# Nikhil-AI-Labs/image-super-resolution-2

Measured on AMD Instinct MI355X. Metric: output MPix/s at x4 SR (256->1024), higher is better.
Workload: dtype bf16 (bf16 MFMA operands, fp32 accumulate, fp32 activations in HBM); 1 GPU; FreqFusion x4 full 3-expert forward (HAT-L + DAT + NAFNet-SR + fusion stack), one 256x256 LR tile -> 1024x1024 per step per GPU (BASELINE configs[1]); seeded synthetic weights (172.3 M params), 1/f-noise tiles; tile=256, parallelism=tile-sharded x1, weights RCCL-broadcast once (0.0 ms), no per-tile collectives, launch=hipGraph replay, tiles_in_flight=2

## Files before the change

image-super-resolution-2_amd/build.py:

```python
from __future__ import annotations

import os
import subprocess
import sys
from concurrent.futures import ThreadPoolExecutor

HERE = os.path.dirname(os.path.abspath(__file__))
CSRC = os.path.join(HERE, "csrc")
LIB = os.path.join(HERE, "libff_hip.so")
SOURCES = ["ff_runtime.hip", "conv_gemm.hip", "conv_gemm_bf16.hip", "conv3x3_halo.hip", "sgfn_tail.hip", "ocab_attn.hip", "conv3x3_small.hip", "attention.hip", "attention_bf16.hip", "win_attn_fused.hip", "chan_qkv.hip", "token_mlp.hip", "token_linear.hip", "naf_fused.hip", "norm_pool.hip", "dwconv.hip", "elementwise.hip",
           "resample.hip", "freq.hip", "fusion_ops.hip", "metrics.hip", "train_ops.hip", "sr_losses.hip", "ff_executor.hip"]
HIPCC = os.environ.get("HIPCC", "/opt/rocm/bin/hipcc")
FLAGS = ["--offload-arch=gfx950", "-O3", "-fPIC", "-std=c++17", "-Wall", "-Wno-unused-function", "-I" + os.path.join(HERE, "build")]


def _stale() -> bool:
    if not os.path.exists(LIB):
        return True
    t = os.path.getmtime(LIB)
    deps = [os.path.join(CSRC, f) for f in os.listdir(CSRC)] + [os.path.join(HERE, "..", "include", "ff_kernels.h")]
    return any(os.path.getmtime(d) > t for d in deps)


def gen_dispatch(path: str) -> None:
    from .lib import parse_header
    protos = {n: p for n, p in parse_header().items() if p[1] and p[1][-1] == "void*" and p[0] == "int"
              and n not in ("ff_forward", "ff_create", "ff_upload")}
    names = sorted(protos)
    out = ["// generated by build.py from include/ff_kernels.h -- do not edit", f"#define FF_DISPATCH_COUNT {len(names)}",
           "static const char* const FF_DISPATCH_NAMES[FF_DISPATCH_COUNT] = {" + ", ".join(f'"{n}"' for n in names) + "};"]
    def kinds(n):
        ks = []
        for i, ty in enumerate(protos[n][1]):
            if i == len(protos[n][1]) - 1:
                ks.append("S")
            elif ty.endswith("*"):
                ks.append("P")
            elif ty in ("float", "double"):
                ks.append("F")
            else:
                ks.append("I")
        return "".join(ks)
    out.append("static const char* const FF_DISPATCH_KINDS[FF_DISPATCH_COUNT] = {" + ", ".join(f'"{kinds(n)}"' for n in names) + "};")
    for n in names:
        out.append(f'extern "C" int {n}(' + ", ".join(protos[n][1]) + ");")
    out.append("static int ff_dispatch(int id, const FFVal* v) {\n  switch (id) {")
    for k, n in enumerate(names):
        args = []
        for i, ty in enumerate(protos[n][1]):
            if ty.endswith("*"):
                args.append(f"({ty})v[{i}].p")
            elif ty in ("float", "double"):
                args.append(f"({ty})v[{i}].f")
            else:
                args.append(f"({ty})v[{i}].i")
        out.append(f"    case {k}: return {n}(" + ", ".join(args) + ");")
    out.append('    default: ff_set_error("ff_dispatch: bad entry point id %d", id); return FF_ERR_ARG;\n  }\n}')
    txt = "\n".join(out) + "\n"
    if not os.path.exists(path) or open(path).read() != txt:
        open(path, "w").write(txt)


def build(force: bool = False, verbose: bool = False) -> str:
# ... 27 lines not shown
```

image-super-resolution-2_amd/experts.py:

```python
from __future__ import annotations

import os
from typing import Dict, List, Optional

import torch

from . import ops
from .prep import (pack_conv, pack_dw, bn_scale_shift, fold_bn_after_conv, pack_token_mlp, pack_token_linear, pack_naf_ffn,
                   pack_win_attn, pack_win_rel, pack_token_projmlp, pack_chan_qkv, pack_token_linear_gated, pack_rel_overlap)

T = torch.Tensor
SD = Dict[str, T]
RGB_MEAN = (0.4488, 0.4371, 0.4040)


def _ceil_to(n: int, m: int) -> int:
    return (n + m - 1) // m * m


class _Weights:

    def __init__(self, sd: SD, dev, prefix: str):
        self.sd, self.dev, self.p = sd, dev, prefix

    def __call__(self, name: str) -> T:
        return self.sd[self.p + name].to(self.dev, torch.float32).contiguous()

    def conv(self, name: str) -> T:
        return pack_conv(self(name + ".weight"))

    def opt(self, name: str) -> Optional[T]:
        k = self.p + name
        return self.sd[k].to(self.dev, torch.float32).contiguous() if k in self.sd else None


def _tl(blk: dict, key: str) -> dict:
    pk = blk.get(key + "_tl")
    if pk is None:
        pk = blk[key + "_tl"] = pack_token_linear(blk[key][0], blk[key][1])
    return pk


_BF16_ROWS = os.environ.get("FF_BF16_ROWS", "1") != "0"
_OCAB_V2 = os.environ.get("FF_OCAB_V2", "1") != "0"
_SGFN_TAIL = os.environ.get("FF_SGFN_TAIL", "1") != "0"


def _fast() -> bool:
    return ops.fused_modes()


_WIN_FUSED = os.environ.get("FF_WIN_FUSED", "1") != "0"
_PROJ_MLP = os.environ.get("FF_PROJ_MLP", "1") != "0"
_LN_ON_LOAD = os.environ.get("FF_LN_ON_LOAD", "1") != "0"
_CHAN_FUSED = os.environ.get("FF_CHAN_FUSED", "1") != "0"
_GATED_PROJ = os.environ.get("FF_GATED_PROJ", "1") != "0"


def _pm(blk: dict) -> dict:
    pk = blk.get("projmlp_pk")
    if pk is None:
# ... 365 lines not shown
            x = ops.conv2d(x, *self.after, ksize=(3, 3), pad=(1, 1), res=feat)
        x = ops.conv2d(x, *self.before_up, ksize=(3, 3), pad=(1, 1), act="lrelu")
        x = ops.conv2d(x, *self.up0, ksize=(3, 3), pad=(1, 1), shuffle=2)
        x = ops.conv2d(x, *self.up2, ksize=(3, 3), pad=(1, 1), shuffle=2)
        sr = ops.conv2d(x, *self.last, ksize=(3, 3), pad=(1, 1))
        return ops.nhwc_to_nchw(sr, 4 * h, 4 * w, clamp01=True)


class NafnetHIP:

    def __init__(self, sd: SD, dev, prefix: str = "expert_ensemble.nafnet.nafnet.", enc=(2, 2, 4, 8), mid: int = 12,
                 dec=(2, 2, 2, 2)):
        w = _Weights(sd, dev, prefix)
        self.dev, self.enc_n, self.mid_n, self.dec_n = dev, enc, mid, dec

        def blk(q):
            def c1(n):
                wt = w(q + n + ".weight")
                return wt.reshape(wt.shape[0], wt.shape[1]).contiguous(), w(q + n + ".bias")
            return dict(n1=(w(q + "norm1.weight"), w(q + "norm1.bias")), n2=(w(q + "norm2.weight"), w(q + "norm2.bias")),
                        c1=c1("conv1"), c2=(pack_dw(w(q + "conv2.weight")), w(q + "conv2.bias")), c3=c1("conv3"),
                        sca=c1("sca.1"), c4=c1("conv4"), c5=c1("conv5"),
                        beta=w(q + "beta").reshape(-1).contiguous(), gamma=w(q + "gamma").reshape(-1).contiguous())

        self.intro = (w.conv("intro"), w("intro.bias"))
        self.ending = (w.conv("ending"), w("ending.bias"))
        self.encs = [[blk(f"encoders.{l}.{b}.") for b in range(n)] for l, n in enumerate(enc)]
        self.mids = [blk(f"middle_blks.{b}.") for b in range(mid)]
        self.decs = [[blk(f"decoders.{l}.{b}.") for b in range(n)] for l, n in enumerate(dec)]
        self.downs = [(w.conv(f"downs.{l}"), w(f"downs.{l}.bias")) for l in range(len(enc))]
        self.ups = [w(f"ups.{l}.0.weight").reshape(w(f"ups.{l}.0.weight").shape[0], -1).contiguous() for l in range(len(dec))]

    def _padded_input(self, B: int, Hp: int, Wp: int, dev) -> T:
        return ops.persistent_zeros(id(self), "naf_in", (B, Hp, Wp, 3), dev)

    def __del__(self):
        try:
            ops.drop_persistent(owner=id(self))
        except Exception:
            pass

    def block(self, x: T, k: dict) -> T:
        c = x.shape[-1]
        flash = _fast() and c in (64, 128)
        if flash and _NAF_FRONT and c == 64:
            g, pooled = ops.naf_front(x, _tl(k, "c1"), k["n1"][0], k["n1"][1], *k["c2"])
        else:
            if flash:
                t = ops.token_linear(x, _tl(k, "c1"), gamma=k["n1"][0], beta=k["n1"][1], eps=1e-6)
            else:
                t = ops.linear(ops.layernorm(x, *k["n1"], eps=1e-6), *k["c1"])
            g, pooled = ops.dwconv3_gate_pool(t, *k["c2"])
        sca = ops.vec_mlp(pooled, *k["sca"], None)
        nf = ops.gemm_mode() != "f32"
        if nf:
            y = ops.linear(g, *k["c3"], res=x, mul=k["beta"], kmul=sca.reshape(-1))
        else:
            w3 = ops.mix2(k["c3"][0], ca=sca.reshape(-1))
            y = ops.linear(g, w3, k["c3"][1], res=x, mul=k["beta"], dynamic_w=True)
        if flash:
            if "ffn_pk" not in k:
                k["ffn_pk"] = pack_naf_ffn(k["c4"][0], k["c4"][1], k["c5"][0], k["c5"][1])
            return ops.naf_ffn(y, k["ffn_pk"], k["n2"][0], k["n2"][1], k["gamma"])
        if nf:
            if "c4i" not in k:
                w4, b4 = k["c4"]
                k["c4i"] = (torch.stack((w4[:c], w4[c:]), dim=1).reshape(2 * c, -1).contiguous(),
                            torch.stack((b4[:c], b4[c:]), dim=1).reshape(-1).contiguous())
            g = ops.linear(ops.layernorm(y, *k["n2"], eps=1e-6), *k["c4i"], gate_pairs=True)
        else:
            t = ops.linear(ops.layernorm(y, *k["n2"], eps=1e-6), *k["c4"])
            g = ops.fma3(None, t[..., :c], t[..., c:])
        return ops.linear(g, *k["c5"], res=y, mul=k["gamma"])

    def forward(self, lr: T, taps: Optional[dict] = None, feats: Optional[dict] = None) -> T:
        _, _, h, w = lr.shape
        H, W = 4 * h, 4 * w
        m = 2 ** len(self.enc_n)
        Hp, Wp = _ceil_to(H, m), _ceil_to(W, m)
        inp = self._padded_input(1, Hp, Wp, lr.device)
        ops.resize(lr, (H, W), mode="bicubic", scale_factor=4.0, layout="nchw", out=inp)
        x = ops.conv2d(inp, *self.intro, ksize=(3, 3), pad=(1, 1))
        skips = []
        for lvl, blks in enumerate(self.encs):
            for b, k in enumerate(blks):
                x = self.block(x, k)
                if taps is not None and lvl == 0:
                    taps[f"naf.enc0.b{b}"] = x
            skips.append(x)
            x = ops.conv2d(x, *self.downs[lvl], ksize=(2, 2), stride=(2, 2), pad=(0, 0))
        for k in self.mids:
            x = self.block(x, k)
        if taps is not None:
            taps["naf.mid"] = x
        for lvl, blks in enumerate(self.decs):
            x = ops.conv2d(x, self.ups[lvl], None, shuffle=2, res=skips[-1 - lvl])
            for k in blks:
                x = self.block(x, k)
        if feats is not None:
            feats["nafnet"] = x
        x = ops.conv2d(x, *self.ending, ksize=(3, 3), pad=(1, 1), res=inp)
        return ops.nhwc_to_nchw(x, H, W, clamp01=True)
```

image-super-resolution-2_amd/ops.py:

```python
from __future__ import annotations

from typing import Dict, Optional, Tuple

import torch

from . import lib as _lib

ACT = {None: 0, "none": 0, "gelu": 1, "relu": 2, "lrelu": 3, "sigmoid": 4}
T = torch.Tensor

_PROF = None
_META = [0.0, 0.0]


def _note(flops: float = 0.0, nbytes: float = 0.0):
    _META[0] += flops
    _META[1] += nbytes


def _numel(*ts) -> float:
    return float(sum(t.numel() * (t.element_size() / 4.0) for t in ts if t is not None))


def _instrument(fn):
# ... 544 lines not shown
        slo, shi = stats_range
        stats = torch.empty((rows, 2), device=x.device, dtype=torch.float32)
        sp = stats.data_ptr()
    _lib.check(_L().ff_token_linear(xp, ldx, out.data_ptr(), ldo, rows, K, pk["kpad"], N, pk["nt"], _ptr(gamma), _ptr(beta), float(eps),
                                    pk["w"].data_ptr(), _ptr(pk["b"]), ACT[act], rp, ldr, r2p, ldr2, _ptr(res2_scale), xnp, ldxn,
                                    sp, slo, shi, float(stats_eps), _nterms(), _stream()))
    _note(2.0 * rows * N * K, 4.0 * (rows * K * (2 if want_xn else 1) + rows * N * (1 + (res is not None) + (res2 is not None))))
    if stats is not None:
        return out, stats
    return (out, xn) if want_xn else out


def dwconv3_gate_pool(t: T, w_tap: T, bias: T):
    tp, ldi, B, H, W, C2 = _nhwc(t, "dwconv3_gate_pool.t")
    if B != 1 or C2 % 2 or tuple(w_tap.shape) != (9, C2):
        raise _lib.FFError("dwconv3_gate_pool: expects B == 1, [9, 2C] tap-major weights")
    C = C2 // 2
    out = torch.empty((1, H, W, C), device=t.device, dtype=torch.float32)
    pooled = torch.empty((1, C), device=t.device, dtype=torch.float32)
    nwork = int(_L().ff_dwconv3_gate_pool_workspace(C))
    work = torch.empty(nwork, device=t.device, dtype=torch.float32)
    _lib.check(_L().ff_dwconv3_gate_pool(tp, ldi, out.data_ptr(), C, H, W, C, w_tap.data_ptr(), bias.data_ptr(), pooled.data_ptr(),
                                         work.data_ptr(), nwork, _stream()))
    _note(2.0 * H * W * C2 * 9, 4.0 * H * W * (C2 + C))
    return out, pooled


def naf_front(x: T, pk: dict, ln_g: T, ln_b: T, w_tap: T, dw_bias: T, eps: float = 1e-6):
    xp, ldx, B, H, W, C = _nhwc(x, "naf_front.x")
    if B != 1 or C not in (64, 128) or pk["N"] != 2 * C or pk["K"] != C or pk["kpad"] != C or tuple(w_tap.shape) != (9, 2 * C):
        raise _lib.FFError("naf_front: expects B == 1, C in (64, 128), conv1 packed as [2C, C], [9, 2C] tap-major weights")
    out = torch.empty((1, H, W, C), device=x.device, dtype=torch.float32)
    pooled = torch.empty((1, C), device=x.device, dtype=torch.float32)
    nwork = int(_L().ff_naf_front_workspace(H, W, C))
    work = torch.empty(nwork, device=x.device, dtype=torch.float32)
    _lib.check(_L().ff_naf_front(xp, ldx, H, W, C, ln_g.data_ptr(), ln_b.data_ptr(), float(eps), pk["w"].data_ptr(), pk["b"].data_ptr(),
                                 w_tap.data_ptr(), dw_bias.data_ptr(), out.data_ptr(), C, pooled.data_ptr(), work.data_ptr(), nwork,
                                 _nterms(), _stream()))
    _note(2.0 * H * W * 2 * C * (C + 9), 4.0 * H * W * 2 * C)
    return out, pooled


def naf_ffn(y: T, pk: dict, ln_g: T, ln_b: T, out_scale: T, eps: float = 1e-6) -> T:
    yp, ldy, rows, C = rows_view(y, "naf_ffn.y")
    if C != pk["C"]:
        raise _lib.FFError("naf_ffn: channel mismatch")
    out = torch.empty(tuple(y.shape), device=y.device, dtype=torch.float32)
    _lib.check(_L().ff_naf_ffn(yp, ldy, out.data_ptr(), C, rows, C, ln_g.data_ptr(), ln_b.data_ptr(), float(eps), pk["w"].data_ptr(),
                               pk["b4"].data_ptr(), pk["b5"].data_ptr(), out_scale.data_ptr(), _nterms(), _stream()))
    _note(2.0 * rows * C * 3 * C, 8.0 * rows * C)
    return out


def layernorm(x: T, gamma: T, beta: T, eps: float = 1e-5, out: Optional[T] = None) -> T:
    xp, ldi, rows, C = rows_view(x, "layernorm.x")
    if out is None:
        out = empty_like_rows(x)
    op, ldo, orows, oc = rows_view(out, "layernorm.out")
    if orows != rows or oc != C or gamma.numel() != C or beta.numel() != C:
        raise _lib.FFError("layernorm: shape mismatch")
    _lib.check(_L().ff_layernorm(xp, ldi, op, ldo, rows, C, gamma.data_ptr(), beta.data_ptr(), float(eps), _stream()))
    _note(0.0, 8.0 * rows * C)
    return out


def pool_partials(x: T):
    xp, ld, B, H, W, C = _nhwc(x, "pool_partials.x")
    if B != 1 or not _POOL_MLP:
        return pool_mean(x)
    P = H * W
    rows = int(_L().ff_pool_partial_rows(P))
    part = torch.empty((rows, C), device=x.device, dtype=torch.float32)
    _lib.check(_L().ff_pool_partials(xp, ld, P, C, part.data_ptr(), part.numel(), _stream()))
    return PoolPartials(part, C, 1.0 / float(P))


def pool_mean(x: T) -> T:
    xp, ld, B, H, W, C = _nhwc(x, "pool_mean.x")
    P = H * W
    nwork = int(_L().ff_pool_mean_workspace(B, P, C))
    work = torch.empty(nwork, device=x.device, dtype=torch.float32)
    out = torch.empty((B, C), device=x.device, dtype=torch.float32)
    _lib.check(_L().ff_pool_mean(xp, ld, B, P, C, out.data_ptr(), work.data_ptr(), nwork, _stream()))
    _note(0.0, 4.0 * B * P * C)
    return out


def vec_mlp(v, W1: T, b1: Optional[T], act1, W2: Optional[T] = None, b2: Optional[T] = None, act2=None,
            post: float = 1.0) -> T:
    if isinstance(v, PoolPartials):
        if W2 is not None and W1.shape[0] <= 64 and v.C <= 512 and _POOL_MLP:
            if W1.shape[1] != v.C or W2.shape[1] != W1.shape[0]:
                raise _lib.FFError("vec_mlp: weight shape mismatch")
            out = torch.empty((1, W2.shape[0]), device=v.part.device, dtype=torch.float32)
            _lib.check(_L().ff_pool_vec_mlp(v.part.data_ptr(), v.part.shape[0], v.part.shape[1], v.inv_count, v.C, W1.data_ptr(), _ptr(b1),
                                            W1.shape[0], ACT[act1], W2.data_ptr(), _ptr(b2), W2.shape[0], ACT[act2], float(post),
                                            out.data_ptr(), None, _stream()))
            return out
        v = v.mean()
    B, Cin = v.shape
    Ch = W1.shape[0]
    Cout = W2.shape[0] if W2 is not None else Ch
    if W1.shape[1] != Cin or (W2 is not None and W2.shape[1] != Ch):
        raise _lib.FFError("vec_mlp: weight shape mismatch")
    out = torch.empty((B, Cout), device=v.device, dtype=torch.float32)
    _lib.check(_L().ff_vec_mlp(v.data_ptr(), B, Cin, W1.data_ptr(), _ptr(b1), Ch, ACT[act1], _ptr(W2), _ptr(b2), Cout,
# ... 314 lines not shown

def band_mha_core(qkv: T, P: int, nbands: int, heads: int) -> T:
    _chk(qkv, "band_mha_core.qkv")
    E = qkv.shape[-1] // 3
    out = torch.empty((P * nbands, E), device=qkv.device, dtype=torch.float32)
    _lib.check(_L().ff_band_mha_core(qkv.data_ptr(), out.data_ptr(), P, nbands, heads, _stream()))
    return out


def band_weight(x: T, att: T, imp: T) -> T:
    out = torch.empty_like(x)
    P = x.numel() // x.shape[-1]
    _lib.check(_L().ff_band_weight(x.data_ptr(), att.data_ptr(), imp.data_ptr(), out.data_ptr(), P, x.shape[-1] // 3, _stream()))
    return out


def freq_guidance(b3: T) -> T:
    P = b3.numel() // 9
    out = torch.empty(tuple(b3.shape[:-1]) + (3,), device=b3.device, dtype=torch.float32)
    _lib.check(_L().ff_freq_guidance(b3.data_ptr(), out.data_ptr(), P, _stream()))
    return out


def dynamic_gates(graw: T, dif: T) -> T:
    P = graw.numel() // 3
    out = torch.empty_like(graw)
    _lib.check(_L().ff_dynamic_gates(graw.data_ptr(), dif.data_ptr(), out.data_ptr(), P, _stream()))
    return out


def fuse_blend(experts9: T, hier3: T, guide3: T, gates3: T, dif1: T) -> T:
    _, Hh, Wh, _ = experts9.shape
    _, Hl, Wl, _ = guide3.shape
    out = torch.empty((1, Hh, Wh, 3), device=experts9.device, dtype=torch.float32)
    _lib.check(_L().ff_fuse_blend(experts9.data_ptr(), hier3.data_ptr(), guide3.data_ptr(), gates3.data_ptr(), dif1.data_ptr(),
                                  out.data_ptr(), Hh, Wh, Hl, Wl, _stream()))
    return out


def tile_accum(tile: T, wy: T, wx: T, acc: T, wsum: T, sy: int, sx: int):
    for t_, n_ in ((tile, "tile"), (wy, "wy"), (wx, "wx"), (acc, "acc"), (wsum, "wsum")):
        _chk(t_, "tile_accum." + n_)
    _, C, th, tw = tile.shape
    _, _, H, W = acc.shape
    _lib.check(_L().ff_tile_accum(tile.contiguous().data_ptr(), C, th, tw, wy.data_ptr(), wx.data_ptr(), acc.data_ptr(),
                                  wsum.data_ptr(), H, W, sy, sx, _stream()))


def tile_normalize(acc: T, wsum: T):
    _, C, H, W = acc.shape
    _lib.check(_L().ff_tile_normalize(acc.data_ptr(), wsum.data_ptr(), C, H, W, _stream()))


for _n in ("conv2d", "sgfn_tail", "ocab_attn", "linear", "win_attn_fused", "token_projmlp", "token_linear_gated", "token_mlp", "token_linear", "pixel_mlp", "dwconv3_gate_pool", "naf_front", "naf_ffn", "window_attn", "layernorm", "pool_mean", "vec_mlp", "dwconv2d", "dwconv3x3_ln", "mix2", "fma3", "affine",
           "nchw_to_nhwc", "nhwc_to_nchw", "resize", "avgpool2", "dct8_bands", "dwt_pass", "fft_bands", "chan_attn_weights", "chan_qkv_attn",
           "band_mha_core", "band_weight", "freq_guidance", "dynamic_gates", "fuse_blend", "tile_accum", "tile_normalize"):
    globals()[_n] = _instrument(globals()[_n])
```

image-super-resolution-2_amd/prep.py:

```python
from __future__ import annotations

from typing import Dict, Optional, Tuple

import torch

T = torch.Tensor


def pack_conv(w: T) -> T:
    co, ci, kh, kw = w.shape
    return w.permute(0, 2, 3, 1).reshape(co, kh * kw * ci).contiguous()


def pack_dw(w: T) -> T:
    c, _, kh, kw = w.shape
    return w.reshape(c, kh * kw).t().contiguous()


def pack_sgfn_fc2(w2: T) -> T:
    n, k = w2.shape
    assert n <= 192
    ht = (k + 31) // 32
    t = torch.zeros(192, ht * 32, device=w2.device, dtype=torch.float32)
    t[:n, :k] = w2
# ... 67 lines not shown
    if nterms == 3:
        rows[..., wk:2 * wk] = lo.reshape(nblk, bn, 9, nchunk, nh, wk).permute(0, 3, 2, 4, 1, 5)
    rec = bn * rw
    slot = (rec * 2 + 1023) // 1024 * 1024
    img = torch.zeros(nblk * nchunk * 9 * nh, slot // 2, device=wp.device, dtype=torch.bfloat16)
    img[:, :rec] = rows.reshape(nblk * nchunk * 9 * nh, rec)
    return img.contiguous()


def pack_rel_overlap(table: T, wh: int, kh: int) -> T:
    rel_w = wh + kh - 1
    n = rel_w * rel_w
    if tuple(table.shape[:1]) != (n,):
        raise ValueError(f"pack_rel_overlap: expected a table of {n} rows, got {tuple(table.shape)}")
    a = wh - kh + 1
    m = ((wh - 1) - a) * (rel_w + 1)
    idx = (torch.arange(n, device=table.device) - m) % n
    return table[idx].t().contiguous()


def pack_token_linear(w: T, b: Optional[T]) -> dict:
    N, K = w.shape
    assert K <= 192
    kpad = 64 if K <= 64 else (128 if K <= 128 else 192)
    nt = (N + 31) // 32
    wp = torch.zeros(nt * 32, kpad, device=w.device)
    wp[:N, :K] = w
    hi, lo = split_bf16(wp.reshape(nt, 32 * kpad))
    bp = None
    if b is not None:
        bp = torch.zeros(nt * 32, device=w.device)
        bp[:N] = b
    return dict(nt=nt, K=K, kpad=kpad, N=N, w=torch.stack([hi, lo], dim=1).contiguous(), b=bp)


def pack_naf_ffn(w4: T, b4: T, w5: T, b5: T) -> dict:
    C = w5.shape[0]
    assert C in (64, 128) and tuple(w4.shape) == (2 * C, C) and tuple(w5.shape) == (C, C)
    gt = C // 32
    pos = torch.arange(32)
    src = ((pos & ~12) | ((pos & 4) << 1) | ((pos & 8) >> 1)).to(w4.device)
    recs = []
    for g in range(gt):
        a = w4[32 * g:32 * g + 32].reshape(-1)
        b = w4[C + 32 * g:C + 32 * g + 32].reshape(-1)
        w5t = w5[:, 32 * g:32 * g + 32][:, src].reshape(-1)
        ah, al = split_bf16(a)
        bh, bl = split_bf16(b)
        wh, wl = split_bf16(w5t)
        recs.append(torch.cat([ah, al, bh, bl, wh, wl]))
    return dict(C=C, w=torch.stack(recs).contiguous(), b4=b4.contiguous(), b5=b5.contiguous())


def win_rel_stride(ww: int) -> int:
    return {8: 40, 16: 48, 32: 64}[ww]


def pack_win_rel(rel: T, wh: int, ww: int) -> T:
    heads = rel.shape[0]
    rows, cols, st = 2 * wh - 1, 2 * ww - 1, win_rel_stride(ww)
    out = torch.zeros(heads, rows, st, device=rel.device, dtype=torch.float32)
    out[:, :, :cols] = rel.reshape(heads, rows, cols)
    return out.contiguous()


def pack_win_attn(wqkv: T, bqkv: Optional[T], heads: int, d: int, scale: float) -> dict:
    C3, K = wqkv.shape
    C = C3 // 3
    assert K <= 192 and heads * d == C and d <= 32
    dev = wqkv.device
    wt = torch.zeros(3 * heads, 32, 192, device=dev)
    bt = torch.zeros(3 * heads, 32, device=dev)
    for g in range(heads):
        for j in range(3):
            rows = slice(j * C + g * d, j * C + (g + 1) * d)
            sc = scale if j == 0 else 1.0
            wt[3 * g + j, :d, :K] = wqkv[rows] * sc
            if bqkv is not None:
                bt[3 * g + j, :d] = bqkv[rows] * sc
    hi, lo = split_bf16(wt.reshape(3 * heads, 32 * 192))
    return dict(w=torch.stack([hi, lo], dim=1).contiguous(), b=bt.reshape(-1).contiguous(), heads=heads, d=d, K=K)


def projmlp_k_perm() -> T:
    k = torch.arange(192)
    st, hh, j = k // 16, (k % 16) // 8, k % 8
    return 32 * (st // 2) + 8 * (2 * (st % 2) + j // 4) + 4 * hh + (j % 4)


def pack_token_projmlp(wp: T, bp: T, w1: T, b1: T, w2: T, b2: T) -> dict:
    hidden, K = w1.shape
    assert K <= 192 and tuple(wp.shape) == (K, K)
    w1p = torch.zeros(hidden, 192, device=w1.device)
    w1p[:, :K] = w1
    w1perm = w1p[:, projmlp_k_perm().to(w1.device)].contiguous()
    mlp = pack_token_mlp(w1perm, b1, w2, b2)
    mlp["K"] = K
    return dict(proj=pack_token_linear(wp, bp), mlp=mlp)


def pack_chan_qkv(wqkv: T, bqkv: Optional[T], heads: int = 6, d: int = 30) -> dict:
    C3, K = wqkv.shape
    C = C3 // 3
    assert C == heads * d == 180 and K <= 192
    dev = wqkv.device
    wt = torch.zeros(18, 32, 192, device=dev)
# ... 47 lines not shown
```

include/ff_kernels.h:

```cpp
#ifndef FF_KERNELS_H
#define FF_KERNELS_H
#ifdef __cplusplus
extern "C" {
#endif

#define FF_ACT_NONE 0
#define FF_ACT_GELU 1
#define FF_ACT_RELU 2
#define FF_ACT_LRELU 3
#define FF_ACT_SIGMOID 4

const char* ff_last_error(void);
int ff_abi_version(void);
int ff_device_cu_count(void);

int ff_conv2d(const float* in, const float* w, const float* bias, const float* mul, const float* res, float* out,
              int B, int H, int W, int Cin, int ldi, int Ho, int Wo, int Cout, int ldo, int ldr, int KH, int KW,
              int sy, int sx, int py, int px, int act, float alpha, int shuffle, int tile_hint, void* stream);

int ff_conv2d_bf16s(const float* in, const void* w_hi, const void* w_lo, int Kp, int Cp, const float* bias, const float* mul,
                    const float* res, float* out, int B, int H, int W, int Cin, int ldi, int Ho, int Wo, int Cout,
                    int ldo, int ldr, int KH, int KW, int sy, int sx, int py, int px, int act, float alpha, int shuffle,
                    int nterms, int tile_hint, const float* kmul, void* stream);
int ff_split_bf16(const float* w, int N, int K, int Kp, int Cin, int Cp, void* hi, void* lo, void* stream);
// ... 3 lines not shown


int ff_window_attn(const float* qkv, int ldq, int q_off, int k_off, int v_off, float* out, int ldo, int o_off,
                   const float* biasT, int B, int H, int W, int Hp, int Wp, int wh, int ww, int kh, int kw,
                   int shift_h, int shift_w, int use_mask, int heads, int d, float scale, void* stream);

int ff_window_attn_bf16s(const float* qkv, int ldq, int q_off, int k_off, int v_off, float* out, int ldo, int o_off,
                         const float* biasT, int B, int H, int W, int Hp, int Wp, int wh, int ww, int kh, int kw,
                         int shift_h, int shift_w, int use_mask, int heads, int d, float scale, int nterms, const float* rel_table,
                         void* stream);

int ff_token_projmlp(const float* att, int lda, const float* x, int ldx, const float* c2, int ldc, const float* c2_scale,
                     float* out, int ldo, long long M, int K, int hidden_tiles, const void* proj_tiles,
                     const float* proj_bias_padded, const float* gamma, const float* beta, float eps,
                     const void* mlp_tiles, const float* b1_padded, const float* b2, int nterms, int io_bf16, void* stream);

int ff_win_attn_fused(const float* x, int ldx, float* out, int ldo, int o_off, const float* gamma, const float* beta,
                      float eps, const void* w_tiles, const float* bias_padded, const float* rel_padded, int rel_rows,
                      int rel_stride, int B, int H, int W, int Hp, int Wp, int wh, int ww, int shift_h, int shift_w,
                      int use_mask, int head0, int nheads, int d, int K, int zero_pad_tokens, float* xn_out, int ldxn,
                      float* v_out, int ldv, int v_off, int nterms, int out_bf16, int xn_bf16, void* stream);

int ff_token_mlp(const float* x, int ldx, float* out, int ldo, long long M, int K, int hidden_tiles, int N,
                 const float* gamma, const float* beta, float eps, const void* w_tiles, const float* b1_padded,
                 const float* b2, int nterms, void* stream);

long long ff_conv3x3_halo_weight_bytes(int Cout, int Cin, int bn, int nterms);
long long ff_conv3x3_halo_pool_rows(int B, int H, int W, int Cout, int bn, int nterms);
int ff_pool_finish(const float* part, int rows, int ld, int C, float inv_count, float* out, void* stream);
int ff_conv3x3_halo(const float* in, int ldi, const void* w_img, int bn, const float* bias, const float* mul,
                    const float* res, int ldr, float* out, int ldo, int B, int H, int W, int Cin, int Cout,
                    int act, float alpha, int shuffle, float* pool_partials, int nterms, int io_bf16, void* stream);

int ff_token_linear(const float* x, int ldx, float* out, int ldo, long long M, int K, int kpad, int N, int n_tiles,
                    const float* gamma, const float* beta, float eps, const void* w_tiles, const float* bias_padded,
                    int act, const float* res, int ldr, const float* res2, int ldr2, const float* res2_scale,
                    float* xn_out, int ldxn, float* stats_out, int stat_lo,
                    int stat_hi, float stat_eps, int nterms, void* stream);

int ff_token_linear_gated(const float* x, int ldx, const float* x2, int ldx2, const float* cm, const float* gw1t, const float* gb1,
                          const float* gw2, float gb2, float* out, int ldo, long long M, int K, int N, int n_tiles,
                          const void* w_tiles, const float* bias_padded, const float* res, int ldr, int nterms, void* stream);

long long ff_dwconv3_gate_pool_workspace(int C);
int ff_dwconv3_gate_pool(const float* in, int ldi, float* out, int ldo, int H, int W, int C, const float* w_tapmajor,
                         const float* bias, float* pooled, float* work, long long work_floats, void* stream);

long long ff_naf_front_workspace(int H, int W, int C);
int ff_naf_front(const float* x, int ldx, int H, int W, int C, const float* ln_gamma, const float* ln_beta, float eps,
                 const void* w1_tiles, const float* b1, const float* dw_tapmajor, const float* dw_bias, float* out, int ldo,
                 float* pooled, float* work, long long work_floats, int nterms, void* stream);
int ff_naf_ffn(const float* y, int ldy, float* out, int ldo, long long M, int C, const float* gamma_ln, const float* beta_ln,
               float eps, const void* w_tiles, const float* b4, const float* b5, const float* out_scale, int nterms, void* stream);

int ff_layernorm(const float* in, int ldi, float* out, int ldo, long long rows, int C, const float* gamma,
                 const float* beta, float eps, void* stream);

int ff_pool_mean(const float* in, int ld, int B, long long P, int C, float* out, float* work, long long work_floats,
                 void* stream);
long long ff_pool_mean_workspace(int B, long long P, int C);

int ff_vec_mlp(const float* in, int B, int Cin, const float* W1, const float* b1, int Ch, int act1, const float* W2,
               const float* b2, int Cout, int act2, float post, float* out, void* stream);

int ff_pool_partial_rows(long long P);
int ff_pool_partials(const float* in, int ld, long long P, int C, float* part, long long part_floats, void* stream);

int ff_pool_vec_mlp(const float* part, int rows, int ld, float inv_count, int Cin, const float* W1, const float* b1, int Ch,
                    int act1, const float* W2, const float* b2, int Cout, int act2, float post, float* out, float* pooled_out,
                    void* stream);

int ff_ocab_attn(const float* qkv, int ldq, int q_off, int k_off, int v_off, float* out, int ldo, int o_off,
                 const float* rel_rotated, int B, int H, int W, int heads, int d, int ws, int ows, float scale, int out_bf16, void* stream);

int ff_sgfn_tail(const float* h, int ldh, int c2, const float* stats, const float* gamma, const float* beta,
                 const float* dw_tapmajor, const float* dw_bias, const void* fc2_tiles, int hidden_tiles, const float* b2,
                 const float* res, int ldr, float* out, int ldo, int B, int H, int W, int N, void* stream);

int ff_dwconv2d(const float* in, int ldi, float* out, int ldo, int B, int H, int W, int C, int Ho, int Wo,
                const float* w_tapmajor, const float* bias, int KH, int KW, int sy, int sx, int py, int px,
                const float* post_scale, const float* post_shift, int act, const float* mul_in, int ldm, void* stream);

int ff_dwconv3x3_ln(const float* in, int ldi, float* out, int ldo, int B, int H, int W, int C, const float* w_tapmajor,
                    const float* bias, const float* stats, const float* gamma, const float* beta, const float* mul_in, int ldm,
                    void* stream);

int ff_mix2(float* out, int ldo, const float* a, int lda, const float* b, int ldb, long long rows, int C, float ka,
            float kb, const float* ca, const float* cb, const float* pa, int ldpa, const float* pb, int ldpb,
            int clamp01, void* stream);
int ff_fma3(float* out, int ldo, const float* a, int lda, const float* b, int ldb, const float* c, int ldc,
            long long rows, int C, float alpha, void* stream);
int ff_affine(float* out, int ldo, const float* in, int ldi, long long rows, int C, const float* scale,
              const float* shift, int act, void* stream);

int ff_pixel_mlp(const float* in, int ldi, long long P, int C, int hidden, const float* W1, const float* b1, int act1,
                 const float* w2, float b2, int act2, float* out, void* stream);

int ff_u8hwc_to_f32nchw(const unsigned char* in, float* out, int H, int W, void* stream);
int ff_f32nchw_to_u8hwc(const float* in, unsigned char* out, int H, int W, void* stream);

int ff_nchw_to_nhwc(const float* in, float* out, int B, int C, int H, int W, int Hp, int Wp, int ldo,
                    const float* add, int pad_mode, void* stream);
int ff_nhwc_to_nchw(const float* in, float* out, int B, int C, int H, int W, int Hs, int Ws, int ldi,
                    const float* add, int clamp01, void* stream);

int ff_tile_accum(const float* tile, int C, int th, int tw, const float* wy, const float* wx, float* acc, float* wsum,
// ... 121 lines not shown
```

Baseline: 24.67 output MPix/s.

## Fuse NAFNet block tail (SCA conv, residual, LN, gated FFN) into one MFMA kernel

Adds a persistent HIP kernel that fuses the NAFNet block's channel-attention-scaled 1x1 conv, beta residual, layernorm, gated FFN and gamma residual. The intermediate y tensor no longer makes an HBM round trip, and the separate linear and naf_ffn launches are dropped. All weights are packed into bf16 MFMA fragments held in LDS, and the next tile's loads are prefetched into registers. It runs only in plain bf16 gemm mode with the fast path on, at the cost of heavy register and LDS pressure and a single-term bf16 contraction for the c3 conv.

```diff
diff --git a/image-super-resolution-2_amd/build.py b/image-super-resolution-2_amd/build.py
--- a/image-super-resolution-2_amd/build.py
+++ b/image-super-resolution-2_amd/build.py
@@ -8,7 +8,7 @@
 HERE = os.path.dirname(os.path.abspath(__file__))
 CSRC = os.path.join(HERE, "csrc")
 LIB = os.path.join(HERE, "libff_hip.so")
-SOURCES = ["ff_runtime.hip", "conv_gemm.hip", "conv_gemm_bf16.hip", "conv3x3_halo.hip", "sgfn_tail.hip", "ocab_attn.hip", "conv3x3_small.hip", "attention.hip", "attention_bf16.hip", "win_attn_fused.hip", "chan_qkv.hip", "token_mlp.hip", "token_linear.hip", "naf_fused.hip", "norm_pool.hip", "dwconv.hip", "elementwise.hip",
+SOURCES = ["ff_runtime.hip", "conv_gemm.hip", "conv_gemm_bf16.hip", "conv3x3_halo.hip", "sgfn_tail.hip", "ocab_attn.hip", "conv3x3_small.hip", "attention.hip", "attention_bf16.hip", "win_attn_fused.hip", "chan_qkv.hip", "token_mlp.hip", "token_linear.hip", "naf_fused.hip", "naf_tail.hip", "norm_pool.hip", "dwconv.hip", "elementwise.hip",
            "resample.hip", "freq.hip", "fusion_ops.hip", "metrics.hip", "train_ops.hip", "sr_losses.hip", "ff_executor.hip"]
 HIPCC = os.environ.get("HIPCC", "/opt/rocm/bin/hipcc")
 FLAGS = ["--offload-arch=gfx950", "-O3", "-fPIC", "-std=c++17", "-Wall", "-Wno-unused-function", "-I" + os.path.join(HERE, "build")]
diff --git a/image-super-resolution-2_amd/csrc/naf_tail.hip b/image-super-resolution-2_amd/csrc/naf_tail.hip
--- /dev/null
+++ b/image-super-resolution-2_amd/csrc/naf_tail.hip
@@ -0,0 +1,255 @@
+#include "ff_common.h"
+
+typedef __bf16 bf16x8 __attribute__((ext_vector_type(8)));
+
+struct NafTailParams {
+  const float* g; const float* x; float* out;
+  const __bf16* w;
+  const float* sca;
+  const float* b3;
+  const float* beta;
+  const float* gamma_ln; const float* beta_ln;
+  const float* b4;
+  const float* b5;
+  const float* oscale;
+  long long M;
+  int ldg, ldx, ldo;
+  int ntiles;
+  float eps;
+};
+
+template <int KS, int NW>
+__global__ __launch_bounds__(NW * 64, (KS == 4 ? 2 : 1)) void naf_tail_kernel(NafTailParams p) {
+  constexpr int C = 16 * KS, GT = C / 32, NTO = C / 32;
+  constexpr int NT = NW * 64;
+  constexpr int CPP = KS == 4 ? 64 : 32, NPASS = C / CPP, XROW = CPP + 4;
+  constexpr int LPR = CPP / 4, RPI = 64 / LPR, LPP = 32 / RPI, FPP = CPP / 16;
+  constexpr bool EARLY = KS == 8;
+  constexpr int WPIECES = 4 * C * C / 8;
+  constexpr int F4 = NTO * KS, F5 = F4 + 2 * GT * KS;
+  extern __shared__ __attribute__((aligned(16))) unsigned char smem[];
+  const bf16x8* Wl = reinterpret_cast<const bf16x8*>(smem);
+  float* cs = reinterpret_cast<float*>(smem + 8 * C * C);
+  const int tid = threadIdx.x, lane = tid & 63, wid = __builtin_amdgcn_readfirstlane(tid >> 6);
+  const int l31 = lane & 31, hh = lane >> 5;
+  const int rr = lane / LPR, cq = (lane % LPR) * 4;
+  float* xs = cs + 9 * C + wid * (32 * XROW);
+
+  f32x4 tg[NPASS][LPP], tx[NPASS][LPP];
+  const unsigned og = (unsigned)(rr * p.ldg + cq), ox = (unsigned)(rr * p.ldx + cq);
+  auto issue = [&](long long tok0) {
+    const float* gp = p.g + tok0 * p.ldg;
+    const float* xp = p.x + tok0 * p.ldx;
+    if (tok0 + 32 <= p.M) {
+#pragma unroll
+      for (int pass = 0; pass < NPASS; ++pass)
+#pragma unroll
+        for (int j = 0; j < LPP; ++j) {
+          tg[pass][j] = *reinterpret_cast<const f32x4*>(gp + (long long)(RPI * j) * p.ldg + CPP * pass + og);
+          tx[pass][j] = *reinterpret_cast<const f32x4*>(xp + (long long)(RPI * j) * p.ldx + CPP * pass + ox);
+        }
+    } else {
+#pragma unroll
+      for (int pass = 0; pass < NPASS; ++pass)
+#pragma unroll
+        for (int j = 0; j < LPP; ++j) {
+          const bool ok = tok0 + RPI * j + rr < p.M;
+          const f32x4 a = *reinterpret_cast<const f32x4*>(ok ? gp + (long long)(RPI * j) * p.ldg + CPP * pass + og : p.g);
+          const f32x4 b = *reinterpret_cast<const f32x4*>(ok ? xp + (long long)(RPI * j) * p.ldx + CPP * pass + ox : p.x);
+          tg[pass][j] = ok ? a : (f32x4){0.f, 0.f, 0.f, 0.f};
+          tx[pass][j] = ok ? b : (f32x4){0.f, 0.f, 0.f, 0.f};
+        }
+    }
+  };
+  long long tile = blockIdx.x;
+  issue((tile * NW + wid) * 32);
+
+  for (int i = tid; i < WPIECES; i += NT) reinterpret_cast<uint4*>(smem)[i] = reinterpret_cast<const uint4*>(p.w)[i];
+  for (int i = tid; i < C; i += NT) {
+    cs[i] = p.sca[i]; cs[C + i] = p.b3[i]; cs[2 * C + i] = p.beta[i]; cs[3 * C + i] = p.gamma_ln[i]; cs[4 * C + i] = p.beta_ln[i];
+    cs[5 * C + i] = p.b4[i]; cs[6 * C + i] = p.b4[C + i]; cs[7 * C + i] = p.b5[i]; cs[8 * C + i] = p.oscale[i];
+  }
+  __syncthreads();
+
+  for (; tile < p.ntiles; tile += gridDim.x) {
+    const long long tok0 = (tile * NW + wid) * 32;
+    bf16x8 gb[KS];
+    float v[KS][8];
+#pragma unroll
+    for (int pass = 0; pass < NPASS; ++pass) {
+#pragma unroll
+      for (int j = 0; j < LPP; ++j) *reinterpret_cast<f32x4*>(xs + (RPI * j + rr) * XROW + cq) = tg[pass][j];
+#pragma unroll
+      for (int s4 = 0; s4 < FPP; ++s4) {
+        const int st = FPP * pass + s4, k0 = 16 * st + 8 * hh;
+        const f32x4 a = *reinterpret_cast<const f32x4*>(xs + l31 * XROW + 16 * s4 + 8 * hh);
+        const f32x4 b = *reinterpret_cast<const f32x4*>(xs + l31 * XROW + 16 * s4 + 8 * hh + 4);
+        const f32x4 s0 = *reinterpret_cast<const f32x4*>(cs + k0), s1 = *reinterpret_cast<const f32x4*>(cs + k0 + 4);
+#pragma unroll
+        for (int e = 0; e < 4; ++e) { gb[st][e] = (__bf16)(a[e] * s0[e]); gb[st][4 + e] = (__bf16)(b[e] * s1[e]); }
+      }
+    }
+#pragma unroll
+    for (int pass = 0; pass < NPASS; ++pass) {
+#pragma unroll
+      for (int j = 0; j < LPP; ++j) *reinterpret_cast<f32x4*>(xs + (RPI * j + rr) * XROW + cq) = tx[pass][j];
+#pragma unroll
+      for (int s4 = 0; s4 < FPP; ++s4) {
+        const f32x4 a = *reinterpret_cast<const f32x4*>(xs + l31 * XROW + 16 * s4 + 8 * hh);
+        const f32x4 b = *reinterpret_cast<const f32x4*>(xs + l31 * XROW + 16 * s4 + 8 * hh + 4);
+#pragma unroll
+        for (int e = 0; e < 4; ++e) { v[FPP * pass + s4][e] = a[e]; v[FPP * pass + s4][4 + e] = b[e]; }
+      }
+    }
+    if (EARLY && tile + gridDim.x < p.ntiles) issue(((tile + gridDim.x) * NW + wid) * 32);
+
+#pragma unroll
+    for (int n = 0; n < NTO; ++n) {
+      f32x16 acc;
+#pragma unroll
+      for (int r = 0; r < 16; ++r) acc[r] = 0.f;
+#pragma unroll
+      for (int st = 0; st < KS; ++st) acc = __builtin_amdgcn_mfma_f32_32x32x16_bf16(Wl[(n * KS + st) * 64 + lane], gb[st], acc, 0, 0, 0);
+      unsigned tt[16];
+#pragma unroll
+      for (int r = 0; r < 16; ++r) {
+        const int ch = 32 * n + (r & 3) + 8 * (r >> 2) + 4 * hh;
+        tt[r] = __float_as_uint((acc[r] + cs[C + ch]) * cs[2 * C + ch]);
+      }
+#pragma unroll
+      for (int sp = 0; sp < 2; ++sp)
+#pragma unroll
+        for (int e = 0; e < 4; ++e) {
+          const auto sw = __builtin_amdgcn_permlane32_swap(tt[8 * sp + e], tt[8 * sp + 4 + e], false, false);
+          v[2 * n + sp][e] = __uint_as_float(sw[0]) + v[2 * n + sp][e];
+          v[2 * n + sp][4 + e] = __uint_as_float(sw[1]) + v[2 * n + sp][4 + e];
+        }
+    }
+
+    if (!EARLY && tile + gridDim.x < p.ntiles) issue(((tile + gridDim.x) * NW + wid) * 32);
+
+    bf16x8 xh[KS];
+    {
+      float s = 0.f;
+#pragma unroll
+      for (int st = 0; st < KS; ++st)
+#pragma unroll
+        for (int j = 0; j < 8; ++j) s += v[st][j];
+      s += __shfl_xor(s, 32);
+      const float mean = s / (float)C;
+      float qv = 0.f;
+#pragma unroll
+      for (int st = 0; st < KS; ++st)
+#pragma unroll
+        for (int j = 0; j < 8; ++j) { const float d = v[st][j] - mean; qv += d * d; }
+      qv += __shfl_xor(qv, 32);
+      const float rstd = 1.0f / sqrtf(qv / (float)C + p.eps);
+#pragma unroll
+      for (int st = 0; st < KS; ++st) {
+        const int k0 = 16 * st + 8 * hh;
+        const f32x4 g0 = *reinterpret_cast<const f32x4*>(cs + 3 * C + k0), g1 = *reinterpret_cast<const f32x4*>(cs + 3 * C + k0 + 4);
+        const f32x4 b0 = *reinterpret_cast<const f32x4*>(cs + 4 * C + k0), b1 = *reinterpret_cast<const f32x4*>(cs + 4 * C + k0 + 4);
+#pragma unroll
+        for (int j = 0; j < 8; ++j) {
+          const float f = (v[st][j] - mean) * rstd * (j < 4 ? g0[j & 3] : g1[j & 3]) + (j < 4 ? b0[j & 3] : b1[j & 3]);
+          xh[st][j] = (__bf16)f;
+        }
+      }
+    }
+
+    f32x16 oacc[NTO];
+#pragma unroll
+    for (int n = 0; n < NTO; ++n)
+#pragma unroll
+      for (int r = 0; r < 16; ++r) oacc[n][r] = 0.f;
+
+#pragma unroll
+    for (int g = 0; g < GT; ++g) {
+      f32x16 ha, hb;
+#pragma unroll
+      for (int r = 0; r < 16; ++r) {
+        const int ch = 32 * g + (r & 3) + 8 * (r >> 2) + 4 * hh;
+        ha[r] = cs[5 * C + ch];
+        hb[r] = cs[6 * C + ch];
+      }
+#pragma unroll
+      for (int st = 0; st < KS; ++st) {
+        ha = __builtin_amdgcn_mfma_f32_32x32x16_bf16(Wl[(F4 + (2 * g) * KS + st) * 64 + lane], xh[st], ha, 0, 0, 0);
+        hb = __builtin_amdgcn_mfma_f32_32x32x16_bf16(Wl[(F4 + (2 * g + 1) * KS + st) * 64 + lane], xh[st], hb, 0, 0, 0);
+      }
+      bf16x8 gh[2];
+#pragma unroll
+      for (int s = 0; s < 2; ++s)
+#pragma unroll
+        for (int j = 0; j < 8; ++j) gh[s][j] = (__bf16)(ha[8 * s + j] * hb[8 * s + j]);
+#pragma unroll
+      for (int n = 0; n < NTO; ++n)
+#pragma unroll
+        for (int s = 0; s < 2; ++s)
+          oacc[n] = __builtin_amdgcn_mfma_f32_32x32x16_bf16(Wl[(F5 + (g * NTO + n) * 2 + s) * 64 + lane], gh[s], oacc[n], 0, 0, 0);
+    }
+
+    float* tr = xs;
+#pragma unroll
+    for (int n = 0; n < NTO; ++n) {
+#pragma unroll
+      for (int sp = 0; sp < 2; ++sp)
+#pragma unroll
+        for (int j = 0; j < 8; ++j) tr[l31 * 33 + 16 * sp + 8 * hh + j] = v[2 * n + sp][j];
+      float rv[16];
+#pragma unroll
+      for (int i = 0; i < 16; ++i) rv[i] = tr[(2 * i + hh) * 33 + l31];
+#pragma unroll
+      for (int r = 0; r < 16; ++r) tr[l31 * 33 + (r & 3) + 8 * (r >> 2) + 4 * hh] = oacc[n][r];
+      const int col = n * 32 + l31;
+      const float sc = cs[8 * C + col], bb = cs[7 * C + col];
+      float ov[16];
+#pragma unroll
+      for (int i = 0; i < 16; ++i) ov[i] = (tr[(2 * i + hh) * 33 + l31] + bb) * sc + rv[i];
+      float* op = p.out + (tok0 + hh) * p.ldo + col;
+      if (tok0 + 32 <= p.M) {
+#pragma unroll
+        for (int i = 0; i < 16; ++i) op[(long long)(2 * i) * p.ldo] = ov[i];
+      } else {
+#pragma unroll
+        for (int i = 0; i < 16; ++i)
+          if (tok0 + 2 * i + hh < p.M) op[(long long)(2 * i) * p.ldo] = ov[i];
+      }
+    }
+  }
+}
+
+template <int KS, int NW, int WGPC>
+static int launch_naf_tail(NafTailParams& p, hipStream_t st) {
+  constexpr int C = 16 * KS;
+  constexpr size_t lds = (size_t)8 * C * C + (size_t)9 * C * 4 + (size_t)NW * 32 * ((KS == 4 ? 64 : 32) + 4) * 4;
+  static_assert(lds <= 160 * 1024, "LDS budget");
+  static bool attr_set = false;
+  if (!attr_set) {
+    hipError_t e = hipFuncSetAttribute(reinterpret_cast<const void*>(&naf_tail_kernel<KS, NW>), hipFuncAttributeMaxDynamicSharedMemorySize, (int)lds);
+    if (e != hipSuccess) { ff_set_error("ff_naf_tail: cannot raise dynamic LDS: %s", hipGetErrorString(e)); return FF_ERR_LAUNCH; }
+    attr_set = true;
+  }
+  const long long ntiles = (p.M + NW * 32 - 1) / (NW * 32);
+  if (ntiles >= (1LL << 31)) { ff_set_error("ff_naf_tail: too many rows"); return FF_ERR_ARG; }
+  p.ntiles = (int)ntiles;
+  const long long nblk = ntiles < 256 * WGPC ? ntiles : 256 * WGPC;
+  hipLaunchKernelGGL((naf_tail_kernel<KS, NW>), dim3((unsigned)nblk), dim3(NW * 64), lds, st, p);
+  FF_LAUNCH_CHECK("ff_naf_tail");
+  return FF_OK;
+}
+
+extern "C" int ff_naf_tail(const float* g, int ldg, const float* x, int ldx, float* out, int ldo, long long M, int C,
+                           const float* sca, const float* b3, const float* beta, const float* gamma_ln, const float* beta_ln,
+                           float eps, const void* w_frags, const float* b4, const float* b5, const float* out_scale, void* stream) {
+  FF_CHECK_ARG(g && x && out && sca && b3 && beta && gamma_ln && beta_ln && w_frags && b4 && b5 && out_scale, "ff_naf_tail: null pointer");
+  FF_CHECK_ARG(M > 0 && (C == 64 || C == 128), "ff_naf_tail: C must be 64 or 128");
+  FF_CHECK_ARG(ldg >= C && ldg % 4 == 0 && ldx >= C && ldx % 4 == 0 && ldo >= C, "ff_naf_tail: row strides must be >= C (g, x: multiples of 4)");
+  FF_CHECK_ARG((((uintptr_t)g) & 15) == 0 && (((uintptr_t)x) & 15) == 0 && (((uintptr_t)w_frags) & 15) == 0, "ff_naf_tail: 16-byte alignment required");
+  FF_CHECK_ARG(out != g && out != x, "ff_naf_tail: out must not alias g or x");
+  NafTailParams p;
+  p.g = g; p.x = x; p.out = out; p.w = (const __bf16*)w_frags; p.sca = sca; p.b3 = b3; p.beta = beta; p.gamma_ln = gamma_ln;
+  p.beta_ln = beta_ln; p.b4 = b4; p.b5 = b5; p.oscale = out_scale; p.M = M; p.ldg = ldg; p.ldx = ldx; p.ldo = ldo; p.eps = eps;
+  p.ntiles = 0;
+  return C == 64 ? launch_naf_tail<4, 4, 2>(p, (hipStream_t)stream) : launch_naf_tail<8, 4, 1>(p, (hipStream_t)stream);
+}
diff --git a/image-super-resolution-2_amd/experts.py b/image-super-resolution-2_amd/experts.py
--- a/image-super-resolution-2_amd/experts.py
+++ b/image-super-resolution-2_amd/experts.py
@@ -6,7 +6,7 @@
 import torch
 
 from . import ops
-from .prep import (pack_conv, pack_dw, bn_scale_shift, fold_bn_after_conv, pack_token_mlp, pack_token_linear, pack_naf_ffn,
+from .prep import (pack_conv, pack_dw, bn_scale_shift, fold_bn_after_conv, pack_token_mlp, pack_token_linear, pack_naf_ffn, pack_naf_tail,
                    pack_win_attn, pack_win_rel, pack_token_projmlp, pack_chan_qkv, pack_token_linear_gated, pack_rel_overlap)
 
 T = torch.Tensor
@@ -478,6 +478,10 @@
                 t = ops.linear(ops.layernorm(x, *k["n1"], eps=1e-6), *k["c1"])
             g, pooled = ops.dwconv3_gate_pool(t, *k["c2"])
         sca = ops.vec_mlp(pooled, *k["sca"], None)
+        if flash and ops.gemm_mode() == "bf16":
+            if "tail_pk" not in k:
+                k["tail_pk"] = pack_naf_tail(*k["c3"], *k["c4"], *k["c5"])
+            return ops.naf_tail(g, x, k["tail_pk"], sca.reshape(-1), k["beta"], k["n2"][0], k["n2"][1], k["gamma"])
         nf = ops.gemm_mode() != "f32"
         if nf:
             y = ops.linear(g, *k["c3"], res=x, mul=k["beta"], kmul=sca.reshape(-1))
diff --git a/image-super-resolution-2_amd/ops.py b/image-super-resolution-2_amd/ops.py
--- a/image-super-resolution-2_amd/ops.py
+++ b/image-super-resolution-2_amd/ops.py
@@ -620,6 +620,25 @@
     return out
 
 
+def naf_tail(g: T, x: T, pk: dict, sca: T, beta: T, ln_g: T, ln_b: T, gamma: T, eps: float = 1e-6) -> T:
+    if _GEMM_MODE != "bf16":
+        raise _lib.FFError(f"naf_tail exists for the plain-bf16 contraction mode only, not {_GEMM_MODE!r}")
+    gp, ldg, rows, C = rows_view(g, "naf_tail.g")
+    xp, ldx, xr, xc = rows_view(x, "naf_tail.x")
+    if C != pk["C"] or xr != rows or xc != C or tuple(x.shape) != tuple(g.shape):
+        raise _lib.FFError("naf_tail: shape mismatch")
+    for t_, n_ in ((sca, "sca"), (beta, "beta"), (ln_g, "ln_g"), (ln_b, "ln_b"), (gamma, "gamma")):
+        _chk(t_, "naf_tail." + n_)
+        if t_.numel() != C or not t_.is_contiguous():
+            raise _lib.FFError(f"naf_tail: {n_} must be a contiguous [{C}] vector")
+    out = torch.empty(tuple(x.shape), device=x.device, dtype=torch.float32)
+    _lib.check(_L().ff_naf_tail(gp, ldg, xp, ldx, out.data_ptr(), C, rows, C, sca.data_ptr(), pk["b3"].data_ptr(), beta.data_ptr(),
+                                ln_g.data_ptr(), ln_b.data_ptr(), float(eps), pk["w"].data_ptr(), pk["b4"].data_ptr(),
+                                pk["b5"].data_ptr(), gamma.data_ptr(), _stream()))
+    _note(2.0 * rows * C * 4 * C, 12.0 * rows * C)
+    return out
+
+
 def layernorm(x: T, gamma: T, beta: T, eps: float = 1e-5, out: Optional[T] = None) -> T:
     xp, ldi, rows, C = rows_view(x, "layernorm.x")
     if out is None:
@@ -1040,7 +1059,7 @@
     _lib.check(_L().ff_tile_normalize(acc.data_ptr(), wsum.data_ptr(), C, H, W, _stream()))
 
 
-for _n in ("conv2d", "sgfn_tail", "ocab_attn", "linear", "win_attn_fused", "token_projmlp", "token_linear_gated", "token_mlp", "token_linear", "pixel_mlp", "dwconv3_gate_pool", "naf_front", "naf_ffn", "window_attn", "layernorm", "pool_mean", "vec_mlp", "dwconv2d", "dwconv3x3_ln", "mix2", "fma3", "affine",
+for _n in ("conv2d", "sgfn_tail", "ocab_attn", "linear", "win_attn_fused", "token_projmlp", "token_linear_gated", "token_mlp", "token_linear", "pixel_mlp", "dwconv3_gate_pool", "naf_front", "naf_ffn", "naf_tail", "window_attn", "layernorm", "pool_mean", "vec_mlp", "dwconv2d", "dwconv3x3_ln", "mix2", "fma3", "affine",
            "nchw_to_nhwc", "nhwc_to_nchw", "resize", "avgpool2", "dct8_bands", "dwt_pass", "fft_bands", "chan_attn_weights", "chan_qkv_attn",
            "band_mha_core", "band_weight", "freq_guidance", "dynamic_gates", "fuse_blend", "tile_accum", "tile_normalize"):
     globals()[_n] = _instrument(globals()[_n])
diff --git a/image-super-resolution-2_amd/prep.py b/image-super-resolution-2_amd/prep.py
--- a/image-super-resolution-2_amd/prep.py
+++ b/image-super-resolution-2_amd/prep.py
@@ -143,6 +143,23 @@
     return dict(C=C, w=torch.stack(recs).contiguous(), b4=b4.contiguous(), b5=b5.contiguous())
 
 
+def pack_naf_tail(w3: T, b3: T, w4: T, b4: T, w5: T, b5: T) -> dict:
+    C = w5.shape[0]
+    assert C in (64, 128) and tuple(w3.shape) == (C, C) and tuple(w4.shape) == (2 * C, C) and tuple(w5.shape) == (C, C)
+    pos = torch.arange(32)
+    src = ((pos & ~12) | ((pos & 4) << 1) | ((pos & 8) >> 1)).to(w4.device)
+
+    def frags(w):
+        r, k = w.shape
+        return w.reshape(r // 32, 32, k // 16, 2, 8).permute(0, 2, 3, 1, 4).reshape(-1)
+
+    f4 = torch.stack([torch.stack((w4[32 * g:32 * g + 32], w4[C + 32 * g:C + 32 * g + 32])) for g in range(C // 32)])
+    f5 = torch.stack([w5[:, 32 * g:32 * g + 32][:, src] for g in range(C // 32)])
+    img = torch.cat([frags(w3), frags(f4.reshape(-1, C)), frags(f5.reshape(-1, 32))]).to(torch.bfloat16).contiguous()
+    assert img.numel() == 4 * C * C
+    return dict(C=C, w=img, b3=b3.contiguous(), b4=b4.contiguous(), b5=b5.contiguous())
+
+
 def win_rel_stride(ww: int) -> int:
     return {8: 40, 16: 48, 32: 64}[ww]
 
diff --git a/include/ff_kernels.h b/include/ff_kernels.h
--- a/include/ff_kernels.h
+++ b/include/ff_kernels.h
@@ -79,6 +79,10 @@
                  float* pooled, float* work, long long work_floats, int nterms, void* stream);
 int ff_naf_ffn(const float* y, int ldy, float* out, int ldo, long long M, int C, const float* gamma_ln, const float* beta_ln,
                float eps, const void* w_tiles, const float* b4, const float* b5, const float* out_scale, int nterms, void* stream);
+
+int ff_naf_tail(const float* g, int ldg, const float* x, int ldx, float* out, int ldo, long long M, int C, const float* sca,
+                const float* b3, const float* beta, const float* gamma_ln, const float* beta_ln, float eps, const void* w_frags,
+                const float* b4, const float* b5, const float* out_scale, void* stream);
 
 int ff_layernorm(const float* in, int ldi, float* out, int ldo, long long rows, int C, const float* gamma,
                  const float* beta, float eps, void* stream);
```

New measurement: 25.03 output MPix/s, median of 6. +1.5%, better.
